# AppleHolic/pytorch_sound

Hardware: AMD Instinct MI355X
Metric: audio-sec/s STFT+mel+fwd/bwd (higher is better)
Workload: dtype bf16; 1 GPU; configs[1]: Conv1d separator (4 x ResBlock1, C=256, on 513-bin magnitude), 22.05 kHz, STFT 1024/256, 80 mel, batch 32 x 2 s per GPU, Adam, bf16 autocast; global_batch=32, parallelism=dp1, model_params=5520386

## Files before the change

include/psnd.h:

```cpp
#ifndef PSND_H
#define PSND_H

#include <stdint.h>
#include <stddef.h>

#ifdef __cplusplus
extern "C" {
#endif

#define PSND_OK 0
#define PSND_E_ARG (-1)
#define PSND_E_SHAPE (-2)
#define PSND_E_HIP (-3)
#define PSND_E_UNSUPPORTED (-4)

#define PSND_FRAMING_CENTER 0
#define PSND_FRAMING_HIFIGAN 1
#define PSND_FRAMING_NONE 2

int psnd_version(void);
const char *psnd_last_error(void);
#ifdef PSND_LAB
void psnd_env_refresh(void);
#endif
// ... 121 lines not shown
int psnd_convtr1d_cl_fwd(const void *xa, const void *wf, const float *bias_rep, int64_t N, int Lp, int L, int HP, int Cip, int Cr,
                         int stride, int padding, int LpO, int HPO, float act_slope, void *out_raw, void *out_act, void *stream);
int psnd_convtr1d_cl_wgrad_splits(int64_t N, int Lp, int Cip, int Cr, int stride);
int psnd_convtr1d_cl_bwd(const void *g_raw, const void *g_act, const void *act, float act_slope, const void *wb, const void *xa,
                         int64_t N, int Lp, int L, int HP, int Cip, int Cr, int stride, int padding, int LpO, int HPO, void *gx,
                         void *g_eff, float *gw_part, void *stream);
int psnd_convtr1d_wnorm_bwd(const float *gw_part, int splits, const float *v, const float *g, int Cin, int Cout, int K, int stride,
                            int Cr, int Cip, float *gv, float *gg, void *stream);
int psnd_cl_mean_act_fwd(const void *a, const void *b, const void *c, const void *d, int count, float slope, void *out, int64_t n,
                         void *stream);
int psnd_cl_mean_act_bwd(const void *g, const void *y, int count, float slope, void *gin, int64_t n, void *stream);
int psnd_cl_sum2(const void *const *a, int na, void *out_a, const void *const *b, int nb, void *out_b, int64_t n, void *stream);
int psnd_cl_colsum_splits(int64_t rows, int C);
int psnd_cl_colsum(const void *g, int64_t rows, int C, int Lp, int lo, int hi, float *part, float *out, void *stream);
int psnd_conv1d_prep_multi(const void *descs_dev, int n, int total_blocks, int max_row, int which, void *stream);
#define PSND_WNORM_MAX 32
typedef struct psnd_wnorm_desc {
    const float *gw_part, *gbias_part;
    const float *v, *g;
    float *gv, *gg, *gbias;
    int splits, Cout, Cin, k, Cb, Ca;
} psnd_wnorm_desc;
int psnd_conv1d_wnorm_bwd_multi(const psnd_wnorm_desc *descs, int n, void *stream);
int psnd_conv1d_cl_bwd(const void *G1, const void *G2, const void *GM, float g2_slope, const void *wb, const void *xa,
                       int64_t N, int Lp, int L, int HP, int Ca, int Cb, int k, int pad, int dil, void *gx, void *g_out,
                       const void *gx_mask, float gx_mask_slope, const void *gx_res, float *gw_part, float *gbias_part,
                       void *stream);
int psnd_conv1d_cl_pair_bwd_supported(int C, int k, int pad2, int dil2, int pad1, int dil1);
int psnd_conv1d_cl_pair_bwd_splits(int64_t N, int Lp, int C, int k);
int psnd_conv1d_cl_pair_bwd(const void *G, const void *wb2, const void *M1, float m1_slope, void *g_mid, const void *wb1, const void *M2,
                            float m2_slope, const void *res, int64_t N, int Lp, int L, int HP, int C, int k, int pad2, int dil2,
                            int pad1, int dil1, void *gx, const void *xa_a, float *gw_a, float *gb_a, const void *G_b,
                            const void *xa_b, int off_b, int dstep_b, float *gw_b, float *gb_b, void *stream);
int psnd_conv1d_wnorm_bwd(const float *gw_part, const float *gbias_part, int splits, const float *v, const float *g,
                          int Cout, int Cin, int k, int Cb, int Ca, float *gv, float *gg, float *gbias, void *stream);
int psnd_to_cl(const float *x, int64_t N, int C, int64_t T, int Lp, int HP, int Cp, int preop, void *out, void *stream);
int psnd_from_cl_tanh(const void *x, int64_t N, int C, int64_t T, int Lp, int HP, int Cp, float *out, void *stream);
int psnd_to_cl_tanh_bwd(const float *g, const float *out_fwd, int64_t N, int C, int64_t T, int Lp, int HP, int Cp, void *gx, void *stream);
int psnd_from_cl(const void *x, int64_t N, int C, int64_t T, int Lp, int HP, int Cp, float *out, void *stream);
int psnd_mask_head_fwd(const void *y, const float *mag, int64_t N, int C, int64_t T, int Lp, int HP, int Cp, float *est,
                       void *stream);
int psnd_mask_head_bwd(const float *gest, const float *mag, const void *y, int64_t N, int C, int64_t T, int Lp, int HP, int Cp,
                       void *gy, void *stream);

int psnd_linear1x1_fwd(const float *x, const float *w, const float *bias, int64_t N, int Cin, int Cout, int64_t T, int relu, int bf16,
                       float *y, void *stream);
// ... 96 lines not shown
```

pytorch_sound_amd/_lib.py:

```python
import ctypes
import os
import numpy as np

_HERE = os.path.dirname(os.path.abspath(__file__))
LIB_PATH = os.environ.get('PSND_LIB', os.path.join(_HERE, 'libpsnd_hip.so'))

PSND_OK = 0
FRAMING_CENTER = 0
FRAMING_HIFIGAN = 1
FRAMING_NONE = 2
LOG_NONE, LOG_E, LOG_10 = 0, 1, 2

_c = ctypes
_P = _c.c_void_p
_I64 = _c.c_int64
_INT = _c.c_int
_F = _c.c_float
_D = _c.c_double

SIGNATURES = {
    'psnd_version': (_INT, []),
    'psnd_last_error': (_c.c_char_p, []),
    'psnd_event_create': (_P, []),
    'psnd_event_destroy': (_INT, [_P]),
# ... 12 lines not shown
    'psnd_mel_plan_build': (_INT, [_INT, _INT, _P, _P]),
    'psnd_mel_fwd': (_INT, [_P, _I64, _I64, _INT, _INT, _P, _INT, _F, _F, _F, _F, _P, _P, _P]),
    'psnd_mel_bwd': (_INT, [_P, _P, _I64, _I64, _INT, _INT, _P, _INT, _F, _F, _F, _F, _P, _P]),
    'psnd_logmel_fwd': (_INT, [_P, _I64, _I64, _INT, _INT, _INT, _P, _F, _INT, _P, _INT, _F, _F, _F, _F, _P, _P]),
    'psnd_conv1d_cl': (_INT, [_P, _P, _P, _F, _P, _P, _P, _P, _I64, _INT, _INT, _INT, _INT, _INT, _INT, _INT, _INT, _F, _F, _P, _P, _P, _P]),
    'psnd_conv1d_cl_pair_supported': (_INT, [_INT, _INT, _INT, _INT, _INT, _INT]),
    'psnd_conv1d_cl_pair': (_INT, [_P, _P, _P, _P, _F, _F, _P, _P, _P, _P, _F, _P, _I64, _INT, _INT, _INT, _INT, _INT, _INT, _INT, _INT, _INT, _F, _P, _P, _P]),
    'psnd_conv1d_cl_wgrad': (_INT, [_P, _P, _P, _F, _P, _I64, _INT, _INT, _INT, _INT, _INT, _INT, _P, _P, _P, _P]),
    'psnd_conv1d_prep': (_INT, [_P, _P, _P, _INT, _INT, _INT, _INT, _INT, _P, _P, _P, _P]),
    'psnd_conv1d_wnorm_bwd': (_INT, [_P, _P, _INT, _P, _P, _INT, _INT, _INT, _INT, _INT, _P, _P, _P, _P]),
    'psnd_conv1d_cl_bwd': (_INT, [_P, _P, _P, _F, _P, _P, _I64, _INT, _INT, _INT, _INT, _INT, _INT, _INT, _INT, _P, _P, _P, _F, _P, _P, _P, _P]),
    'psnd_conv1d_cl_wgrad_multi_splits': (_INT, [_I64, _INT, _INT, _INT, _INT, _INT]),
    'psnd_conv1d_cl_wgrad_multi': (_INT, [_P, _INT, _I64, _INT, _P]),
    'psnd_nan_flag': (_INT, [_P, _I64, _P, _P]),
    'psnd_conv1d_cl_chain_rows': (_INT, [_INT, _INT, _INT, _P]),
    'psnd_conv1d_cl_chain_plan': (_INT, [_INT, _INT, _INT, _P, _I64, _P]),
    'psnd_conv1d_cl_chain': (_INT, [_P, _P, _P, _INT, _I64, _INT, _INT, _INT, _INT, _INT, _P]),
    'psnd_conv_chain_stats': (None, [_P]),
    'psnd_conv1d_cl_pair_bwd_supported': (_INT, [_INT, _INT, _INT, _INT, _INT, _INT]),
    'psnd_conv1d_cl_pair_bwd_splits': (_INT, [_I64, _INT, _INT, _INT]),
    'psnd_conv1d_cl_pair_bwd': (_INT, [_P, _P, _P, _F, _P, _P, _P, _F, _P, _I64, _INT, _INT, _INT, _INT, _INT, _INT, _INT, _INT, _INT, _P, _P, _P, _P,
                                       _P, _P, _INT, _INT, _P, _P, _P]),
    'psnd_conv1d_wnorm_bwd_multi': (_INT, [_P, _INT, _P]),
    'psnd_conv1d_prep_multi': (_INT, [_P, _INT, _INT, _INT, _INT, _P]),
    'psnd_conv1d_cl_wgrad_splits': (_INT, [_I64, _INT, _INT, _INT, _INT]),
    'psnd_mask_head_l1_blocks': (_I64, [_I64, _I64, _INT]),
    'psnd_masked_l1_blocks': (_I64, [_I64]),
    'psnd_masked_l1_fwd': (_INT, [_P, _P, _P, _I64, _INT, _I64, _P, _P, _P, _P]),
    'psnd_masked_l1_bwd': (_INT, [_P, _P, _P, _I64, _INT, _I64, _P, _P, _P, _P, _P]),
    'psnd_to_cl_nfk': (_INT, [_P, _I64, _INT, _I64, _INT, _INT, _INT, _INT, _P, _P]),
    'psnd_mask_head_l1_blocks_nfk': (_I64, [_I64, _I64, _INT]),
    'psnd_mask_head_l1_fwd_nfk': (_INT, [_P, _P, _P, _I64, _INT, _I64, _INT, _INT, _INT, _P, _P, _P]),
    'psnd_mask_head_l1_bwd_nfk': (_INT, [_P, _P, _P, _P, _P, _P, _F, _I64, _INT, _I64, _INT, _INT, _INT, _P, _P]),
    'psnd_mel_fwd_nfk': (_INT, [_P, _I64, _I64, _INT, _INT, _P, _INT, _F, _F, _F, _F, _P, _P, _P]),
    'psnd_mel_bwd_nfk': (_INT, [_P, _P, _I64, _I64, _INT, _INT, _P, _INT, _F, _F, _F, _F, _P, _P]),
    'psnd_mel_l1_fwd_nfk': (_INT, [_P, _I64, _I64, _INT, _INT, _P, _INT, _F, _F, _F, _F, _P, _P, _P, _P]),
    'psnd_mel_l1_bwd_nfk': (_INT, [_P, _P, _P, _F, _I64, _I64, _INT, _INT, _P, _INT, _F, _F, _F, _F, _P, _P]),
    'psnd_mask_head_l1_fwd': (_INT, [_P, _P, _P, _I64, _INT, _I64, _INT, _INT, _INT, _P, _P, _P]),
    'psnd_mask_head_l1_bwd': (_INT, [_P, _P, _P, _P, _P, _P, _F, _I64, _INT, _I64, _INT, _INT, _INT, _P, _P]),
    'psnd_mel_l1_blocks': (_I64, [_I64, _I64, _INT]),
    'psnd_mel_l1_fwd': (_INT, [_P, _I64, _I64, _INT, _INT, _P, _INT, _F, _F, _F, _F, _P, _P, _P, _P]),
    'psnd_mel_l1_bwd': (_INT, [_P, _P, _P, _F, _I64, _I64, _INT, _INT, _P, _INT, _F, _F, _F, _F, _P, _P]),
    'psnd_l1_loss_combine': (_INT, [_P, _P, _P, _INT, _P, _P, _P]),
    'psnd_conv_stats': (_INT, [_P, _INT]),
    'psnd_conv_pair_stats': (_INT, [_P, _INT]),
    'psnd_convtr1d_prep_multi': (_INT, [_P, _INT, _INT, _P]),
# ... 52 lines not shown
    'psnd_l1_loss_blocks': (_I64, [_I64]),
    'psnd_l1_loss_fwd': (_INT, [_P, _P, _I64, _P, _P, _P]),
    'psnd_l1_loss_bwd': (_INT, [_P, _P, _I64, _P, _P, _P, _P]),
    'psnd_l1_loss_sum_fwd': (_INT, [_P, _P, _P, _P, _INT, _P, _P, _P]),
    'psnd_l1_loss_bwd_w': (_INT, [_P, _P, _I64, _P, _D, _P, _P, _P]),
    'psnd_to_cl': (_INT, [_P, _I64, _INT, _I64, _INT, _INT, _INT, _INT, _P, _P]),
    'psnd_from_cl': (_INT, [_P, _I64, _INT, _I64, _INT, _INT, _INT, _P, _P]),
    'psnd_from_cl_tanh': (_INT, [_P, _I64, _INT, _I64, _INT, _INT, _INT, _P, _P]),
    'psnd_to_cl_tanh_bwd': (_INT, [_P, _P, _I64, _INT, _I64, _INT, _INT, _INT, _P, _P]),
}

_lib = None


class PsndError(RuntimeError):
    pass


class WgradDesc(ctypes.Structure):
    _fields_ = [('g', _P), ('xa', _P), ('gw_part', _P), ('gbias_part', _P), ('off0', _INT), ('dstep', _INT),
                ('Ca', _INT), ('Cb', _INT), ('k', _INT), ('splits', _INT)]


class ChainPair(ctypes.Structure):
    _fields_ = [('W1', _P), ('bias1', _P), ('act1_slope', _F), ('mid_out', _P), ('W2', _P), ('bias2', _P),
                ('off1', _INT), ('dstep1', _INT), ('off2', _INT), ('dstep2', _INT), ('act2_slope', _F), ('out_raw', _P), ('out_act', _P),
                ('M1', _P), ('M2', _P), ('m1_slope', _F), ('m2_slope', _F)]


def lib():
    global _lib
    if _lib is None:
        import torch
        if not os.path.exists(LIB_PATH):
            raise PsndError('libpsnd_hip.so not found at %s - run `python -m pytorch_sound_amd._build` '
                            '(there is no CPU / eager fallback)' % LIB_PATH)
        _lib = _load(LIB_PATH)
    return _lib


def _load(path):
    h = ctypes.CDLL(path)
    for name, (res, args) in SIGNATURES.items():
        fn = getattr(h, name)
        fn.restype = res
        fn.argtypes = args
# ... 85 lines not shown
```

pytorch_sound_amd/cl.py:

```python
import ctypes
import os
from pytorch_sound_amd import _switches as _sw
import weakref

import torch

from . import _lib
from ._lib import lib, check, ptr, stream_ptr

ALIGN_C = 32


def round_up(x, m):
    return (x + m - 1) // m * m


class CLShape:

    def __init__(self, N, L, HP):
        self.N, self.L, self.HP = int(N), int(L), int(HP)
        self.Lp = round_up(self.L + 2 * self.HP, 8)

    @property
    def R(self):
# ... 923 lines not shown

        def grad_out(i, v32, g32, Cb):
            gv = gg = gb = None
            if sink is not None and prefs is not None:
                pv, pg, pb = prefs[3 * i:3 * i + 3]
                gv, gg = sink.dest(pv, pv.numel()), sink.dest(pg, pg.numel())
                gb = sink.dest(pb, Cb) if pb is not None else None
                early[i] = [(0, pv) if gv is not None else None, (1, pg) if gg is not None else None,
                            (2, pb) if gb is not None else None]
            gv = torch.empty_like(v32) if gv is None else gv.view_as(v32)
            gg = torch.empty_like(g32) if gg is None else gg.view_as(g32)
            gb = torch.empty(Cb, dtype=torch.float32, device=dev) if gb is None else gb
            return gv, gg, gb

        nsec, sides = _sections(dev, shape.N, shape.N * shape.Lp)
        wstreams = _wgrad_streams(dev) if shape.N * shape.Lp <= 8192 else []
        if wstreams:
            nsec, sides = 1, []
        Nh = shape.N // nsec
        plan = []
        skip = -1
        batch = (nsec == 1 and not wstreams and _pair_enabled() and _sw.lab('PSND_CL_BWD_BATCH', '1') == '1'
                 and shape.N * shape.Lp <= 8192)
        wbatch = []
        own_launch = []
        flush_after = {}
        pair_bwd = (nsec == 1 and not wstreams and not batch and _pair_enabled() and _sw.lab('PSND_CL_PAIR_BWD', '1') != '0'
                    and shape.N * shape.Lp <= 8192)
        lag = None
        with torch.cuda.device(dev):
            g_comb = None
            res_pending = None
            def slabs(i, G1, G2, am, inp, S=None):
                Cout, Cin, k, Ca, Cb, dil, pad, slope = steps[i][:8]
                v32, g32 = saved[5 * i + 3], saved[5 * i + 4]
                if S is None:
                    S = lib().psnd_conv1d_cl_wgrad_splits(Nh, shape.Lp, Ca, Cb, k)
                gw = torch.empty((nsec * S, k, Cb, Ca), dtype=torch.float32, device=dev)
                gbp = torch.empty((nsec * S, Cb), dtype=torch.float32, device=dev)
                gv, gg, gb = grad_out(i, v32, g32, Cb)
                descs[i] = struct.pack('<7Q6i', gw.data_ptr(), gbp.data_ptr(), v32.data_ptr(), g32.data_ptr(), gv.data_ptr(),
                                       gg.data_ptr(), gb.data_ptr(), nsec * S, Cout, Cin, k, Cb, Ca)
                keep.extend([gw, gbp, G1, G2])
                grads[3 * i], grads[3 * i + 1] = gv, gg
                grads[3 * i + 2] = gb[:Cout] if steps[i][9] else None
                return ('w', G1, G2, am, slope, inp, Ca, Cb, k, -pad, dil, gw, gbp, S)
# ... 41 lines not shown
                        wbatch.append((i - 1, g_h, inp1, -pad1, d1))
                        flush_after[id(gx)] = len(wbatch)
                    else:
                        plan.append(('side',) + slabs(i - 1, g_h, None, None, inp1))
                    keep.extend([g_h, gx])
                    res_pending = G
                    g_comb = gx
                    skip = i - 1
                    continue
                if g_comb is None:
                    if g_raw is None and g_act is None:
                        raise _lib.PsndError('CL conv chain backward: no incoming gradient')
                    G1, G2 = g_raw, g_act
                    am = act if g_act is not None else None
                    need_gout = has_res and g_act is not None
                else:
                    G1, G2, am, need_gout = g_comb, None, None, False
                S = lib().psnd_conv1d_cl_wgrad_splits(Nh, shape.Lp, Ca, Cb, k)
                gw = torch.empty((nsec * S, k, Cb, Ca), dtype=torch.float32, device=dev)
                gbp = torch.empty((nsec * S, Cb), dtype=torch.float32, device=dev)
                gv, gg, gb = None, None, None
                g_out = torch.empty((shape.N, shape.Lp, Cb), dtype=torch.bfloat16, device=dev) if need_gout else None
                g_here = g_out if need_gout else G1
                wb_ok = batch and G2 is None and not need_gout and _sw.lab('PSND_CL_BWD_BATCH_ENDS', '0') == '1'
                if i == 0 and not (ctx.needs_input_grad[0] or ctx.needs_input_grad[1]):
                    gx = None
                    if wb_ok:
                        wbatch.append((i, G1, inp, -pad, dil))
                        keep.append(G1)
                        if i > 0:
                            g_comb = gx
                        g_raw = g_act = None
                        continue
                    plan.append((('side',) if wstreams else ()) + ('w', G1, G2, am, slope, inp, Ca, Cb, k, -pad, dil, gw, gbp, S))
                    g_raw = g_act = None
                else:
                    gx = torch.empty((shape.N, shape.Lp, Ca), dtype=torch.bfloat16, device=dev)
                    if i == 0:
                        ep_mask, ep_res = None, None
                    elif role == 'c1':
                        ep_mask, ep_res = inp, res_pending
                    elif role == 'r2':
                        ep_mask, ep_res = inp, g_here
                    else:
                        ep_mask, ep_res = inp, None
                    if wb_ok:
                        plan.append(('b', G1, G2, am, slope, wb, inp, Ca, Cb, k, pad, dil, gx, g_out, ep_mask,
# ... 93 lines not shown
                        check(lib().psnd_conv1d_cl_bwd(q(G1), q(G2), q(am), float(slope), ptr(wb), q(inp), Nh, shape.Lp, shape.L,
                                                       shape.HP, Ca, Cb, k, pad, dil, q(gx), q(g_out), q(ep_mask), ep_slope, q(ep_res),
                                                       None if gw is None else ptr(gw[h * S:(h + 1) * S]),
                                                       None if gbp is None else ptr(gbp[h * S:(h + 1) * S]), st),
                              'psnd_conv1d_cl_bwd')

            st = stream_ptr(dev)
            handed = set()

            def wgrad_batch(part):
                for j0 in range(0, len(part), 32):
                    sub = part[j0:j0 + 32]
                    shp = [(steps[ci][3], steps[ci][4], steps[ci][2]) for ci, _, _, _, _ in sub]
                    main_shape = max(set(shp), key=shp.count)
                    cnt = max(shp.count(main_shape), len(wbatch) // 2) if len(part) < len(wbatch) else shp.count(main_shape)
                    Sb = lib().psnd_conv1d_cl_wgrad_multi_splits(shape.N, shape.Lp, main_shape[0], main_shape[1], main_shape[2], cnt)
                    arr = (_lib.WgradDesc * len(sub))()
                    for d, (ci, G, inp, off0, dstep) in zip(arr, sub):
                        w = slabs(ci, G, None, None, inp, Sb)
                        d.g, d.xa, d.gw_part, d.gbias_part, d.off0, d.dstep = G.data_ptr(), inp.data_ptr(), w[11].data_ptr(), w[12].data_ptr(), off0, dstep
                        d.Ca, d.Cb, d.k, d.splits = steps[ci][3], steps[ci][4], steps[ci][2], Sb
                    check(lib().psnd_conv1d_cl_wgrad_multi(ctypes.addressof(arr), len(sub), shape.N, shape.Lp, st), 'psnd_conv1d_cl_wgrad_multi')

            def finish(convs):
                ds = [descs[ci] for ci in convs]
                for j0 in range(0, len(ds), 32):
                    chunk = ds[j0:j0 + 32]
                    buf = ctypes.create_string_buffer(b''.join(chunk))
                    check(lib().psnd_conv1d_wnorm_bwd_multi(buf, len(chunk), st), 'psnd_conv1d_wnorm_bwd_multi')
                out = []
                for ci in convs:
                    for ent in early.get(ci, ()):
                        if ent is not None:
                            grads[3 * ci + ent[0]] = None
                            out.append(ent[1])
                    handed.add(ci)
                if out:
                    sink.deliver(out)

            if sink is not None and batch and nsec == 1 and not wstreams:
                done_w = 0

                def chunk(part, ready):
                    if part:
                        wgrad_batch(part)
                    finish(ready)

                launches = [e for e in plan if (e[1][-1] if e[0] == 'chainb' else e)[0] == 'pairb']
                L, C = len(launches), max(1, int(HANDOVER_CHUNKS))
                cut = {id(launches[min(L - 1, max(0, round((j + 1) * L / C) - 1))]) for j in range(C - 1)} if L else set()
                ready = []
                for e in plan:
                    run(0, [e])
                    ready += [ci for pe, ci in own_launch if pe is e]
                    last = e[1][-1] if e[0] == 'chainb' else e
                    upto = flush_after.get(id(last[16])) if (last[0] == 'pairb' and id(e) in cut) else None
                    if upto is None:
                        continue
                    part = []
                    if upto is not None and upto > done_w:
                        part = wbatch[done_w:upto]
                        ready += [ci for ci, _, _, _, _ in part]
                        done_w = upto
                    if ready:
                        chunk(part, ready)
                        ready = []
                part = wbatch[done_w:]
                rest = [ci for ci in range(n) if ci not in handed and descs[ci] is not None and ci not in [c for c, _, _, _, _ in part]]
                rest = [ci for ci in rest if ci not in ready]
                if part or rest or ready:
                    chunk(part, ready + rest + [ci for ci, _, _, _, _ in part])
            else:
                _run_sections(dev, nsec, sides, run)
                for sd in set(used):
                    torch.cuda.current_stream(dev).wait_stream(sd)
                wgrad_batch(wbatch)
                finish([ci for ci in range(n) if descs[ci] is not None])
        consume_param_use(ctx)
        return (g_raw, g_act, None, None, None, None, None, None) + tuple(grads)


def _block_node(convs, x, xa, shape, pairs, last_act_slope, want_raw, prep):
    params = []
    for c in convs:
        params += [c.weight_v, c.weight_g, c.bias]
    packs = None if prep is None else _PackList(prep[id(c)] for c in convs)
    if packs is not None:
        packs.owner = prep if isinstance(prep, PrepPacks) else None
    roles = pairs if isinstance(pairs, tuple) else (('c1', 'c2') * (len(convs) // 2) if pairs else ('r2',) * len(convs))
    return ResBlockCL.apply(x, xa, shape, roles, tuple(c.dilation for c in convs), last_act_slope, want_raw, packs, *params)


class _PackList(list):
    owner = None


def _use_block_node(convs, x):
    import os
    return (_sw.lab('PSND_NO_BLOCK_NODE') != '1' and x is not None and len(convs) <= 64
            and all(c.weight_v.shape[0] == c.weight_v.shape[1] for c in convs))


# ... 51 lines not shown
```

pytorch_sound_amd/csrc/psnd_conv.hip:

```cpp
#include "psnd_common.h"
#include "psnd_conv_pair.h"
#include <stdlib.h>
#include <string.h>
#include <atomic>

namespace {

typedef __attribute__((ext_vector_type(8))) short bf16x8;
typedef __attribute__((ext_vector_type(16))) float f32x16;
typedef unsigned short bf16_t;

__device__ __forceinline__ float bf2f(bf16_t v) { return __builtin_bit_cast(float, (unsigned)v << 16); }
__device__ __forceinline__ bf16_t f2bf(float f) {
    unsigned u = __builtin_bit_cast(unsigned, f);
    if ((u & 0x7fffffffu) > 0x7f800000u) return (bf16_t)((u >> 16) | 0x40);
    u += 0x7fffu + ((u >> 16) & 1u);
    return (bf16_t)(u >> 16);
}

typedef __bf16 hwbf16x2 __attribute__((ext_vector_type(2)));
typedef float f32x2_t __attribute__((ext_vector_type(2)));
__device__ __forceinline__ unsigned pack_bf16(float lo, float hi) {
    const f32x2_t v = {lo, hi};
    return __builtin_bit_cast(unsigned, __builtin_convertvector(v, hwbf16x2));
// ... 1235 lines not shown
__global__ __launch_bounds__(1024) void conv_finish_kernel(const float *gw_part, const float *gb_part, int splits, const float *v,
                                                           const float *g, int Cout, int Cin, int k, int Cb, int Ca, float *gv,
                                                           float *gg, float *gbias, unsigned kmagic, unsigned cmagic) {
    extern __shared__ float s_gw[];
    __shared__ float red[32];
    conv_finish_body<MANY>(gw_part, gb_part, splits, v, g, Cin, k, Cb, Ca, gv, gg, gbias, kmagic, cmagic, blockIdx.x, s_gw, red);
}

struct FinishArgs {
    psnd_wnorm_desc d[PSND_WNORM_MAX];
    unsigned kmagic[PSND_WNORM_MAX], cmagic[PSND_WNORM_MAX];
    int blk0[PSND_WNORM_MAX + 1];
    int n;
};
template <bool MANY>
__global__ __launch_bounds__(1024) void conv_finish_multi_kernel(FinishArgs a) {
    extern __shared__ float s_gw[];
    __shared__ float red[32];
    int i = 0;
    while (i + 1 < a.n && (int)blockIdx.x >= a.blk0[i + 1]) ++i;
    const psnd_wnorm_desc &d = a.d[i];
    conv_finish_body<MANY>(d.gw_part, d.gbias_part, d.splits, d.v, d.g, d.Cin, d.k, d.Cb, d.Ca, d.gv, d.gg, d.gbias, a.kmagic[i],
                           a.cmagic[i], (int)blockIdx.x - a.blk0[i], s_gw, red);
}

}

static std::atomic<long long> g_conv_stats[4];
std::atomic<long long> g_conv_pair_stats[4];
extern "C" int psnd_conv_pair_stats(int64_t *out4, int reset) {
    if (out4)
        for (int i = 0; i < 4; ++i) out4[i] = g_conv_pair_stats[i].load();
    if (reset)
        for (int i = 0; i < 4; ++i) g_conv_pair_stats[i].store(0);
    return PSND_OK;
}
extern "C" int psnd_conv_stats(int64_t *out4, int reset) {
    if (out4)
        for (int i = 0; i < 4; ++i) out4[i] = g_conv_stats[i].load();
    if (reset)
        for (int i = 0; i < 4; ++i) g_conv_stats[i].store(0);
    return PSND_OK;
}

static int conv_row_tiles(int64_t R, int Cb, bool with3 = false) {
    const char *fe = PSND_ENV("PSND_CONV_MT");
// ... 567 lines not shown
        if (!d.gw_part || !d.v || !d.g || !d.gv || !d.gg || d.splits < 1 || d.Cout < 1 || d.Cin < 1 || d.k < 1)
            PSND_FAIL(PSND_E_ARG, "conv1d_wnorm_bwd_multi: descriptor %d: null pointer / bad sizes", i);
        const size_t l = sizeof(float) * (size_t)(d.Cin + 1) * d.k;
        if (l > 60 * 1024) PSND_FAIL(PSND_E_SHAPE, "conv1d_wnorm_bwd_multi: Cin*k=%d too large", d.Cin * d.k);
        lds = l > lds ? l : lds;
        a.d[i] = d;
        a.kmagic[i] = (unsigned)((0x100000000ull + (unsigned)d.k - 1) / (unsigned)d.k);
        a.cmagic[i] = (unsigned)((0x100000000ull + (unsigned)d.Cin - 1) / (unsigned)d.Cin);
        a.blk0[i] = total;
        total += d.Cout;
        maxn = d.Cin * d.k > maxn ? d.Cin * d.k : maxn;
        maxsplits = d.splits > maxsplits ? d.splits : maxsplits;
    }
    a.blk0[n] = total;
    const int threads = maxn >= 2048 ? 1024 : 256;
    if (maxsplits > 16)
        hipLaunchKernelGGL(conv_finish_multi_kernel<true>, dim3(total), dim3(1024), lds + 4096, static_cast<hipStream_t>(stream), a);
    else
        hipLaunchKernelGGL(conv_finish_multi_kernel<false>, dim3(total), dim3(threads), lds, static_cast<hipStream_t>(stream), a);
    PSND_CHECK_LAUNCH("conv1d_wnorm_bwd_multi");
    return PSND_OK;
}

namespace {

__global__ __launch_bounds__(256) void convtr_prep_kernel(const float *v, const float *g, const float *bias, int Cin, int Cout, int K, int u,
                                                          int Cr, int Cip, bf16_t *wf, bf16_t *wb, float *bp) {
    __shared__ float red[4];
    const int ci = blockIdx.x, n = Cout * K;
    const float *vr = v + (size_t)ci * n;
    float ss = 0.f;
    for (int i = threadIdx.x; i < n; i += 256) ss += vr[i] * vr[i];
    for (int m = 32; m >= 1; m >>= 1) ss += __shfl_xor(ss, m, 64);
    if ((threadIdx.x & 63) == 0) red[threadIdx.x >> 6] = ss;
    __syncthreads();
    const float scale = g[ci] / __builtin_sqrtf(red[0] + red[1] + red[2] + red[3]);
    const int Nn = u * Cr;
    for (int i = threadIdx.x; i < n; i += 256) {
        const int co = i / K, jk = i - co * K;
        const int tap = jk / u, phi = jk - tap * u;
        const bf16_t w = f2bf(vr[i] * scale);
        wf[pack_index(2, tap, phi * Cr + co, ci, Nn, Cip)] = w;
        wb[pack_index(2, tap, ci, phi * Cr + co, Cip, Nn)] = w;
    }
    if (ci == 0)
        for (int i = threadIdx.x; i < Nn; i += 256) {
// ... 401 lines not shown
```

pytorch_sound_amd/csrc/psnd_core.hip:

```cpp
#include "psnd_common.h"

static thread_local char g_err[512] = "";

void psnd_set_error(const char *fmt, ...) {
    va_list ap;
    va_start(ap, fmt);
    vsnprintf(g_err, sizeof(g_err), fmt, ap);
    va_end(ap);
}

extern "C" int psnd_version(void) { return 137; }

extern "C" const char *psnd_last_error(void) { return g_err; }

#ifdef PSND_LAB
std::atomic<int> g_psnd_env_gen{0};
extern "C" void psnd_env_refresh(void) { g_psnd_env_gen.fetch_add(1, std::memory_order_acq_rel); }
#endif

static inline int64_t pad_of(int n_fft, int hop, int framing) {
    if (framing == PSND_FRAMING_NONE) return 0;
    return framing == PSND_FRAMING_CENTER ? n_fft / 2 : (n_fft - hop) / 2;
}

extern "C" int64_t psnd_frame_count(int64_t T, int n_fft, int hop, int framing) {
    if (T <= 0 || n_fft <= 0 || hop <= 0) return 0;
    const int64_t L = T + 2 * pad_of(n_fft, hop, framing);
    if (L < n_fft) return 0;
    return (L - n_fft) / hop + 1;
}

extern "C" int64_t psnd_frame_sample_index(int64_t f, int m, int64_t T, int n_fft, int hop, int framing) {
    int64_t i = f * hop - pad_of(n_fft, hop, framing) + m;
    if (i < 0) i = -i;
// ... 106 lines not shown
```

Baseline: 97270 audio-s/s.

## Fuse batched conv1d weight-gradient with weight-norm backward in one kernel

Adds a new HIP kernel that computes the split-K weight-gradient slabs for a batch of k=3 channels-last convs with MFMA, then lets the last-arriving block per output tile (found through an atomic counter) run the weight-norm backward reduction in the same launch. Standalone finish blocks handle convs without a wgrad part. The Python backward routes the batched wgrad plus finish work through this path by default when shapes qualify, and also enables batching of end convs under those limits. This removes separate wgrad and wnorm-finish launches and their serialization, at the cost of a persistent counter buffer and shape restrictions.

Result: slower. 93790 audio-s/s, median of 2 (-3.6%).

```diff
diff --git a/include/psnd.h b/include/psnd.h
--- a/include/psnd.h
+++ b/include/psnd.h
@@ -167,6 +167,16 @@
     int splits, Cout, Cin, k, Cb, Ca;
 } psnd_wnorm_desc;
 int psnd_conv1d_wnorm_bwd_multi(const psnd_wnorm_desc *descs, int n, void *stream);
+#define PSND_WGRAD_WN_MAX 28
+typedef struct psnd_wgrad_wn_desc {
+    const void *g, *xa;
+    float *gw_part, *gbias_part;
+    const float *v, *g_w;
+    float *gv, *gg, *gbias;
+    int off0, dstep, Cout, Cin, k, Cb, Ca, splits;
+} psnd_wgrad_wn_desc;
+int psnd_conv1d_cl_wgrad_wn_splits(int64_t N, int Lp, int ci_tiles);
+int psnd_conv1d_cl_wgrad_wn(const psnd_wgrad_wn_desc *d, int n, int64_t N, int Lp, unsigned *counters, void *stream);
 int psnd_conv1d_cl_bwd(const void *G1, const void *G2, const void *GM, float g2_slope, const void *wb, const void *xa,
                        int64_t N, int Lp, int L, int HP, int Ca, int Cb, int k, int pad, int dil, void *gx, void *g_out,
                        const void *gx_mask, float gx_mask_slope, const void *gx_res, float *gw_part, float *gbias_part,
diff --git a/pytorch_sound_amd/_lib.py b/pytorch_sound_amd/_lib.py
--- a/pytorch_sound_amd/_lib.py
+++ b/pytorch_sound_amd/_lib.py
@@ -58,6 +58,8 @@
     'psnd_conv1d_cl_pair_bwd': (_INT, [_P, _P, _P, _F, _P, _P, _P, _F, _P, _I64, _INT, _INT, _INT, _INT, _INT, _INT, _INT, _INT, _INT, _P, _P, _P, _P,
                                        _P, _P, _INT, _INT, _P, _P, _P]),
     'psnd_conv1d_wnorm_bwd_multi': (_INT, [_P, _INT, _P]),
+    'psnd_conv1d_cl_wgrad_wn_splits': (_INT, [_I64, _INT, _INT]),
+    'psnd_conv1d_cl_wgrad_wn': (_INT, [_P, _INT, _I64, _INT, _P, _P]),
     'psnd_conv1d_prep_multi': (_INT, [_P, _INT, _INT, _INT, _INT, _P]),
     'psnd_conv1d_cl_wgrad_splits': (_INT, [_I64, _INT, _INT, _INT, _INT]),
     'psnd_mask_head_l1_blocks': (_I64, [_I64, _I64, _INT]),
@@ -156,6 +158,11 @@
                 ('Ca', _INT), ('Cb', _INT), ('k', _INT), ('splits', _INT)]
 
 
+class WgradWnDesc(ctypes.Structure):
+    _fields_ = [('g', _P), ('xa', _P), ('gw_part', _P), ('gbias_part', _P), ('v', _P), ('g_w', _P), ('gv', _P), ('gg', _P), ('gbias', _P),
+                ('off0', _INT), ('dstep', _INT), ('Cout', _INT), ('Cin', _INT), ('k', _INT), ('Cb', _INT), ('Ca', _INT), ('splits', _INT)]
+
+
 class ChainPair(ctypes.Structure):
     _fields_ = [('W1', _P), ('bias1', _P), ('act1_slope', _F), ('mid_out', _P), ('W2', _P), ('bias2', _P),
                 ('off1', _INT), ('dstep1', _INT), ('off2', _INT), ('dstep2', _INT), ('act2_slope', _F), ('out_raw', _P), ('out_act', _P),
diff --git a/pytorch_sound_amd/cl.py b/pytorch_sound_amd/cl.py
--- a/pytorch_sound_amd/cl.py
+++ b/pytorch_sound_amd/cl.py
@@ -969,6 +969,8 @@
         skip = -1
         batch = (nsec == 1 and not wstreams and _pair_enabled() and _sw.lab('PSND_CL_BWD_BATCH', '1') == '1'
                  and shape.N * shape.Lp <= 8192)
+        wn = (batch and _sw.lab('PSND_CL_WGRAD_WN', '1') == '1'
+              and all(s_[2] == 3 and s_[1] <= 1024 and (s_[10] == 'tail' or (s_[4] <= 256 and 2 * abs(s_[5]) <= 16)) for s_ in steps))
         wbatch = []
         own_launch = []
         flush_after = {}
@@ -1056,7 +1058,8 @@
                 gv, gg, gb = None, None, None
                 g_out = torch.empty((shape.N, shape.Lp, Cb), dtype=torch.bfloat16, device=dev) if need_gout else None
                 g_here = g_out if need_gout else G1
-                wb_ok = batch and G2 is None and not need_gout and _sw.lab('PSND_CL_BWD_BATCH_ENDS', '0') == '1'
+                wb_ok = batch and G2 is None and not need_gout and ((Cb <= 256 and Ca <= 256 and 2 * abs(dil) <= 16) if wn
+                                                                    else _sw.lab('PSND_CL_BWD_BATCH_ENDS', '0') == '1')
                 if i == 0 and not (ctx.needs_input_grad[0] or ctx.needs_input_grad[1]):
                     gx = None
                     if wb_ok:
@@ -1196,8 +1199,26 @@
                         d.Ca, d.Cb, d.k, d.splits = steps[ci][3], steps[ci][4], steps[ci][2], Sb
                     check(lib().psnd_conv1d_cl_wgrad_multi(ctypes.addressof(arr), len(sub), shape.N, shape.Lp, st), 'psnd_conv1d_cl_wgrad_multi')
 
-            def finish(convs):
-                ds = [descs[ci] for ci in convs]
+            S_wn = lib().psnd_conv1d_cl_wgrad_wn_splits(shape.N, shape.Lp, sum((steps[e[0]][3] + 255) // 256 for e in wbatch)) if wn and wbatch else 0
+
+            def wgrad_wn(part, fin):
+                items = [(e[0], e) for e in part] + [(ci, None) for ci in fin]
+                ctr = _wn_counters(dev)
+                for j0 in range(0, len(items), _WN_MAX):
+                    sub = items[j0:j0 + _WN_MAX]
+                    arr = (_lib.WgradWnDesc * len(sub))()
+                    for d, (ci, e) in zip(arr, sub):
+                        if e is not None:
+                            slabs(ci, e[1], None, None, e[2], S_wn)
+                            d.g, d.xa, d.off0, d.dstep = e[1].data_ptr(), e[2].data_ptr(), e[3], e[4]
+                        gw, gbp, v32, g32, gv, gg, gb, S, Cout, Cin, k, Cb, Ca = struct.unpack('<7Q6i', descs[ci])
+                        d.gw_part, d.gbias_part, d.v, d.g_w, d.gv, d.gg, d.gbias = gw, gbp, v32, g32, gv, gg, gb
+                        d.Cout, d.Cin, d.k, d.Cb, d.Ca, d.splits = Cout, Cin, k, Cb, Ca, S
+                    check(lib().psnd_conv1d_cl_wgrad_wn(ctypes.addressof(arr), len(sub), shape.N, shape.Lp, ctr.data_ptr(), st),
+                          'psnd_conv1d_cl_wgrad_wn')
+
+            def finish(convs, launch=True):
+                ds = [descs[ci] for ci in convs] if launch else []
                 for j0 in range(0, len(ds), 32):
                     chunk = ds[j0:j0 + 32]
                     buf = ctypes.create_string_buffer(b''.join(chunk))
@@ -1216,6 +1237,10 @@
                 done_w = 0
 
                 def chunk(part, ready):
+                    if wn:
+                        wgrad_wn(part, [ci for ci in ready if ci not in {e[0] for e in part}])
+                        finish(ready, launch=False)
+                        return
                     if part:
                         wgrad_batch(part)
                     finish(ready)
@@ -1248,10 +1273,29 @@
                 _run_sections(dev, nsec, sides, run)
                 for sd in set(used):
                     torch.cuda.current_stream(dev).wait_stream(sd)
-                wgrad_batch(wbatch)
-                finish([ci for ci in range(n) if descs[ci] is not None])
+                if wn:
+                    wgrad_wn(wbatch, [ci for ci in range(n) if descs[ci] is not None])
+                    finish([ci for ci in range(n) if descs[ci] is not None], launch=False)
+                else:
+                    wgrad_batch(wbatch)
+                    finish([ci for ci in range(n) if descs[ci] is not None])
         consume_param_use(ctx)
         return (g_raw, g_act, None, None, None, None, None, None) + tuple(grads)
+
+
+_WN_MAX = 28
+_WN_COUNTERS = {}
+
+
+def _wn_counters(dev):
+    key = (dev.index, torch.cuda.current_stream(dev).cuda_stream)
+    t = _WN_COUNTERS.get(key)
+    if t is None and torch.cuda.is_current_stream_capturing():
+        t = _WN_COUNTERS.get(dev.index)
+    if t is None:
+        t = _WN_COUNTERS[key] = torch.zeros(4 * _WN_MAX, dtype=torch.int32, device=dev)
+        _WN_COUNTERS.setdefault(dev.index, t)
+    return t
 
 
 def _block_node(convs, x, xa, shape, pairs, last_act_slope, want_raw, prep):
diff --git a/pytorch_sound_amd/csrc/psnd_conv.hip b/pytorch_sound_amd/csrc/psnd_conv.hip
--- a/pytorch_sound_amd/csrc/psnd_conv.hip
+++ b/pytorch_sound_amd/csrc/psnd_conv.hip
@@ -1281,6 +1281,318 @@
     const psnd_wnorm_desc &d = a.d[i];
     conv_finish_body<MANY>(d.gw_part, d.gbias_part, d.splits, d.v, d.g, d.Cin, d.k, d.Cb, d.Ca, d.gv, d.gg, d.gbias, a.kmagic[i],
                            a.cmagic[i], (int)blockIdx.x - a.blk0[i], s_gw, red);
+}
+
+constexpr int WN_MAX = PSND_WGRAD_WN_MAX;
+constexpr int WN_XR = 48;
+constexpr int WN_GP = 96, WN_XP = 288;
+constexpr int WN_STAGE = 32 * WN_GP + WN_XR * WN_XP;
+constexpr int WN_EP = 256 + 4;
+constexpr int kWgradWnLdsBytes = 2 * WN_STAGE * (int)sizeof(bf16_t);
+static_assert(64 * WN_EP * 4 <= kWgradWnLdsBytes, "one tap's 64 x 256 slab tile fits the chunk buffers");
+constexpr int WN_QMAX = 4;
+constexpr int WN_RPP = 2;
+constexpr int WN_WD = 4;
+constexpr int WN_AUX_SC1 = 16;
+struct WgradWnArgs {
+    long long R;
+    int n, nunits, ncompute;
+    int ub0[WN_MAX + 1];
+    int fb0[WN_MAX + 1];
+    int rps[WN_MAX];
+    unsigned *counters;
+    psnd_wgrad_wn_desc d[WN_MAX];
+};
+template <int P>
+__device__ __forceinline__ bf16x8 tr_frag_p(const bf16_t *p0) {
+    const v4s_t a = __builtin_amdgcn_ds_read_tr16_b64_v4i16((v4s_t __attribute__((address_space(3))) *)(p0));
+    const v4s_t b = __builtin_amdgcn_ds_read_tr16_b64_v4i16((v4s_t __attribute__((address_space(3))) *)(p0 + 4 * P));
+    return __builtin_shufflevector(a, b, 0, 1, 2, 3, 4, 5, 6, 7);
+}
+__device__ __forceinline__ void wn_tile(const psnd_wgrad_wn_desc &d, const long long R, const int rps, const int cot, const int cit,
+                                        const int split, bf16_t *sT) {
+    const int tid = threadIdx.x, wave = tid >> 6, lane = tid & 63, li = lane & 31, kg = lane >> 5;
+    const int co0 = cot * 64, ci0 = cit * 256, Ca = d.Ca, Cb = d.Cb;
+    const long long rs = (long long)split * rps, re = min(rs + rps, R);
+    const bool gthr = tid < 256;
+    const int grr = (tid >> 3) & 31, gcg = tid & 7;
+    const int xrr = tid >> 5, xcg = tid & 31;
+    const bool gok = gthr && co0 + 8 * gcg < Cb, xok = ci0 + 8 * xcg < Ca;
+    const bool do_bias = cit == 0 && d.gbias_part != nullptr;
+    const int lo = min(d.off0, d.off0 + 2 * d.dstep), hi = max(d.off0, d.off0 + 2 * d.dstep);
+    const int xrows = 32 + hi - lo;
+    int toff[3];
+#pragma unroll
+    for (int j = 0; j < 3; ++j) toff[j] = d.off0 + j * d.dstep - lo;
+    constexpr unsigned OOB = 0xffffffffu;
+    const __amdgpu_buffer_rsrc_t rG = make_uniform_rsrc(d.g, (int)((size_t)R * Cb * sizeof(bf16_t)));
+    const __amdgpu_buffer_rsrc_t rX = make_uniform_rsrc(d.xa, (int)((size_t)R * Ca * sizeof(bf16_t)));
+    auto ld16 = [&](__amdgpu_buffer_rsrc_t r, unsigned off) __attribute__((always_inline)) {
+        return __builtin_bit_cast(uint4, __builtin_amdgcn_raw_buffer_load_b128(r, (int)off, 0, 0));
+    };
+    f32x16 acc[2][3];
+#pragma unroll
+    for (int m = 0; m < 2; ++m)
+#pragma unroll
+        for (int j = 0; j < 3; ++j)
+#pragma unroll
+            for (int i = 0; i < 16; ++i) acc[m][j][i] = 0.f;
+    float bsum[8] = {0.f, 0.f, 0.f, 0.f, 0.f, 0.f, 0.f, 0.f};
+    uint4 vg[WN_WD], vx[WN_WD][3];
+    auto fetch = [&](auto sc, long long r0) __attribute__((always_inline)) {
+        constexpr int s = decltype(sc)::value;
+        const long long r = r0 + grr;
+        vg[s] = ld16(rG, (r < re && gok) ? (unsigned)(((size_t)r * Cb + co0 + 8 * gcg) * sizeof(bf16_t)) : OOB);
+#pragma unroll
+        for (int u = 0; u < 3; ++u) {
+            const int xi = xrr + 16 * u;
+            const long long rx = r0 + lo + xi;
+            const bool ok = xi < xrows && rx >= 0 && rx < R && xok;
+            vx[s][u] = ld16(rX, ok ? (unsigned)(((size_t)rx * Ca + ci0 + 8 * xcg) * sizeof(bf16_t)) : OOB);
+        }
+    };
+    auto stage = [&](auto sc, bf16_t *sG, bf16_t *sX) __attribute__((always_inline)) {
+        constexpr int s = decltype(sc)::value;
+        if (gthr) {
+            if (do_bias) {
+                const unsigned *pg4 = reinterpret_cast<const unsigned *>(&vg[s]);
+#pragma unroll
+                for (int e = 0; e < 8; ++e) bsum[e] += bf2f((bf16_t)((pg4[e >> 1] >> (16 * (e & 1))) & 0xffff));
+            }
+            *reinterpret_cast<uint4 *>(sG + grr * WN_GP + 8 * gcg) = vg[s];
+        }
+#pragma unroll
+        for (int u = 0; u < 3; ++u) *reinterpret_cast<uint4 *>(sX + (xrr + 16 * u) * WN_XP + 8 * xcg) = vx[s][u];
+    };
+    const int trow = 8 * kg + ((lane & 15) >> 2), tcol = 16 * ((lane >> 4) & 1) + 4 * (lane & 3);
+    const int nchunk = ((int)((re - rs + 31) / 32) + WN_WD - 1) / WN_WD * WN_WD;
+    static_for<0, WN_WD>([&](auto sc) __attribute__((always_inline)) { fetch(sc, rs + 32ll * decltype(sc)::value); });
+    for (int c = 0; c < nchunk; c += WN_WD) {
+        static_for<0, WN_WD>([&](auto sc) __attribute__((always_inline)) {
+            constexpr int s = decltype(sc)::value;
+            const int ch = c + s;
+            bf16_t *sG = sT + (ch & 1) * WN_STAGE, *sX = sG + 32 * WN_GP;
+            stage(sc, sG, sX);
+            __syncthreads();
+            fetch(sc, rs + 32ll * (ch + WN_WD));
+            bf16x8 fa[2][2], fb[2][3];
+#pragma unroll
+            for (int kk = 0; kk < 2; ++kk) {
+#pragma unroll
+                for (int m = 0; m < 2; ++m) fa[kk][m] = tr_frag_p<WN_GP>(sG + (16 * kk + trow) * WN_GP + 32 * m + tcol);
+#pragma unroll
+                for (int j = 0; j < 3; ++j) fb[kk][j] = tr_frag_p<WN_XP>(sX + (16 * kk + trow + toff[j]) * WN_XP + 32 * wave + tcol);
+            }
+#pragma unroll
+            for (int kk = 0; kk < 2; ++kk)
+#pragma unroll
+                for (int m = 0; m < 2; ++m)
+#pragma unroll
+                    for (int j = 0; j < 3; ++j) acc[m][j] = __builtin_amdgcn_mfma_f32_32x32x16_bf16(fa[kk][m], fb[kk][j], acc[m][j], 0, 0, 0);
+        });
+    }
+    __syncthreads();
+    float *sE = reinterpret_cast<float *>(sT);
+    const __amdgpu_buffer_rsrc_t rW = make_uniform_rsrc(d.gw_part, (int)((size_t)d.splits * 3 * Cb * Ca * sizeof(float)));
+#pragma unroll
+    for (int j = 0; j < 3; ++j) {
+        if (j > 0) __syncthreads();
+#pragma unroll
+        for (int m = 0; m < 2; ++m)
+#pragma unroll
+            for (int rg = 0; rg < 16; ++rg) sE[(32 * m + (rg & 3) + 8 * (rg >> 2) + 4 * kg) * WN_EP + 32 * wave + li] = acc[m][j][rg];
+        __syncthreads();
+#pragma unroll
+        for (int u = 0; u < 8; ++u) {
+            const int idx = tid + 512 * u, row = idx >> 6, c4 = 4 * (idx & 63);
+            const int co = co0 + row, ci = ci0 + c4;
+            const bool ok = co < Cb && ci < Ca;
+            const f32x4 v = *reinterpret_cast<const f32x4 *>(sE + row * WN_EP + c4);
+            __builtin_amdgcn_raw_buffer_store_b128(__builtin_bit_cast(u32x4, v), rW,
+                                                   ok ? (int)((((size_t)split * 3 + j) * Cb + co) * Ca + ci) * (int)sizeof(float) : (int)OOB, 0,
+                                                   WN_AUX_SC1);
+        }
+    }
+    __syncthreads();
+    if (do_bias) {
+        float *sb = reinterpret_cast<float *>(sT);
+        if (gthr) {
+#pragma unroll
+            for (int e = 0; e < 8; ++e) {
+                float v = bsum[e];
+#pragma unroll
+                for (int m = 32; m >= 8; m >>= 1) v += __shfl_xor(v, m, 64);
+                if ((lane >> 3) == 0) sb[wave * 64 + 8 * gcg + e] = v;
+            }
+        }
+        __syncthreads();
+        if (tid < 64) {
+            const float v = (sb[tid] + sb[64 + tid]) + (sb[128 + tid] + sb[192 + tid]);
+            const __amdgpu_buffer_rsrc_t rB = make_uniform_rsrc(d.gbias_part, (int)((size_t)d.splits * Cb * sizeof(float)));
+            __builtin_amdgcn_raw_buffer_store_b32(__builtin_bit_cast(unsigned, v), rB,
+                                                  co0 + tid < Cb ? (int)(((size_t)split * Cb + co0 + tid) * sizeof(float)) : (int)OOB, 0, WN_AUX_SC1);
+        }
+    }
+}
+__device__ __forceinline__ void wn_finish(const psnd_wgrad_wn_desc &d, const int cot) {
+    const int tid = threadIdx.x, wave = tid >> 6, lane = tid & 63;
+    const int co0 = cot * 64, S = d.splits, Cin = d.Cin, Ca = d.Ca, Cb = d.Cb;
+    const int nq = (Cin + 255) / 256;
+    const bool v4 = (Cin & 3) == 0;
+    constexpr unsigned OOB = 0xffffffffu;
+    const __amdgpu_buffer_rsrc_t rW = make_uniform_rsrc(d.gw_part, (int)((size_t)S * 3 * Cb * Ca * sizeof(float)));
+    __builtin_amdgcn_fence(__ATOMIC_ACQUIRE, "wavefront");
+    if (tid < 64 && d.gbias && d.gbias_part) {
+        const int co = co0 + tid;
+        const __amdgpu_buffer_rsrc_t rB = make_uniform_rsrc(d.gbias_part, (int)((size_t)S * Cb * sizeof(float)));
+        float b = 0.f;
+        for (int s = 0; s < S; ++s)
+            b += __builtin_bit_cast(float, __builtin_amdgcn_raw_buffer_load_b32(rB, co < d.Cout ? (int)(((size_t)s * Cb + co) * sizeof(float)) : (int)OOB, 0,
+                                                                                 WN_AUX_SC1));
+        if (co < d.Cout) d.gbias[co] = b;
+    }
+    auto load = [&](const int r0, const int q, f32x4 (&G)[WN_RPP][3], float (&V)[WN_RPP][12]) __attribute__((always_inline)) {
+        const int ci = 4 * (lane + 64 * q);
+#pragma unroll
+        for (int r = 0; r < WN_RPP; ++r)
+#pragma unroll
+            for (int j = 0; j < 3; ++j) G[r][j] = f32x4{0.f, 0.f, 0.f, 0.f};
+        for (int s = 0; s < S; s += 2) {
+            f32x4 t[2][WN_RPP][3];
+#pragma unroll
+            for (int h = 0; h < 2; ++h)
+#pragma unroll
+                for (int r = 0; r < WN_RPP; ++r)
+#pragma unroll
+                    for (int j = 0; j < 3; ++j) {
+                        const int co = co0 + r0 + r, sp = s + h < S ? s + h : s;
+                        const bool ok = co < d.Cout && ci < Cin;
+                        t[h][r][j] = __builtin_bit_cast(f32x4, __builtin_amdgcn_raw_buffer_load_b128(
+                                                                   rW, ok ? (int)((((size_t)sp * 3 + j) * Cb + co) * Ca + ci) * (int)sizeof(float) : (int)OOB, 0,
+                                                                   WN_AUX_SC1));
+                    }
+#pragma unroll
+            for (int r = 0; r < WN_RPP; ++r)
+#pragma unroll
+                for (int j = 0; j < 3; ++j) {
+                    G[r][j] += t[0][r][j];
+                    if (s + 1 < S) G[r][j] += t[1][r][j];
+                }
+        }
+#pragma unroll
+        for (int r = 0; r < WN_RPP; ++r) {
+            const int co = co0 + r0 + r;
+            const float *vr = d.v + (size_t)co * Cin * 3 + 3 * ci;
+            if (v4) {
+                const bool ok = co < d.Cout && ci < Cin;
+#pragma unroll
+                for (int u = 0; u < 3; ++u) {
+                    const f32x4 x = ok ? *reinterpret_cast<const f32x4 *>(vr + 4 * u) : f32x4{0.f, 0.f, 0.f, 0.f};
+#pragma unroll
+                    for (int e = 0; e < 4; ++e) V[r][4 * u + e] = x[e];
+                }
+            } else {
+#pragma unroll
+                for (int e = 0; e < 12; ++e) V[r][e] = (co < d.Cout && ci + e / 3 < Cin) ? vr[e] : 0.f;
+            }
+        }
+    };
+    auto store = [&](const int r0, const int q, const f32x4 (&G)[WN_RPP][3], const float (&V)[WN_RPP][12], const float (&gs)[WN_RPP],
+                     const float (&sv)[WN_RPP]) __attribute__((always_inline)) {
+        const int ci = 4 * (lane + 64 * q);
+#pragma unroll
+        for (int r = 0; r < WN_RPP; ++r) {
+            const int co = co0 + r0 + r;
+            if (co >= d.Cout || ci >= Cin) continue;
+            float o[12];
+#pragma unroll
+            for (int e = 0; e < 12; ++e) o[e] = gs[r] * (G[r][e % 3][e / 3] - V[r][e] * sv[r]);
+            float *dst = d.gv + (size_t)co * Cin * 3 + 3 * ci;
+            if (v4) {
+#pragma unroll
+                for (int u = 0; u < 3; ++u) *reinterpret_cast<f32x4 *>(dst + 4 * u) = f32x4{o[4 * u], o[4 * u + 1], o[4 * u + 2], o[4 * u + 3]};
+            } else {
+#pragma unroll
+                for (int e = 0; e < 12; ++e)
+                    if (ci + e / 3 < Cin) dst[e] = o[e];
+            }
+        }
+    };
+    for (int r0 = WN_RPP * wave; r0 < 64; r0 += 8 * WN_RPP) {
+        if (co0 + r0 >= d.Cout) break;
+        f32x4 G[WN_RPP][3];
+        float V[WN_RPP][12], ss[WN_RPP], dot[WN_RPP];
+#pragma unroll
+        for (int r = 0; r < WN_RPP; ++r) ss[r] = 0.f, dot[r] = 0.f;
+        for (int q = 0; q < nq; ++q) {
+            load(r0, q, G, V);
+#pragma unroll
+            for (int r = 0; r < WN_RPP; ++r)
+#pragma unroll
+                for (int e = 0; e < 12; ++e) {
+                    ss[r] = __builtin_fmaf(V[r][e], V[r][e], ss[r]);
+                    dot[r] = __builtin_fmaf(V[r][e], G[r][e % 3][e / 3], dot[r]);
+                }
+        }
+        float gs[WN_RPP], sv[WN_RPP];
+#pragma unroll
+        for (int r = 0; r < WN_RPP; ++r) {
+#pragma unroll
+            for (int m = 32; m >= 1; m >>= 1) {
+                ss[r] += __shfl_xor(ss[r], m, 64);
+                dot[r] += __shfl_xor(dot[r], m, 64);
+            }
+            const int co = co0 + r0 + r;
+            const float inv = 1.f / __builtin_sqrtf(ss[r]);
+            const float dd = dot[r] * inv;
+            gs[r] = co < d.Cout ? d.g_w[co] * inv : 0.f;
+            sv[r] = inv * dd;
+            if (lane == 0 && co < d.Cout) d.gg[co] = dd;
+        }
+        if (nq == 1) {
+            store(r0, 0, G, V, gs, sv);
+        } else {
+            for (int q = 0; q < nq; ++q) {
+                load(r0, q, G, V);
+                store(r0, q, G, V, gs, sv);
+            }
+        }
+    }
+}
+__global__ __launch_bounds__(512, 1) void conv_wgrad_wn_kernel(WgradWnArgs a) {
+    extern __shared__ __attribute__((aligned(16))) bf16_t smem_dyn[];
+    __shared__ int s_last;
+    const int b = (int)blockIdx.x;
+    int i = 0, cot;
+    if (b < a.ncompute) {
+        const int xcd = b & 7, slot = b >> 3;
+        cot = slot & 3;
+        const int u = (slot >> 2) * 8 + xcd;
+        if (u >= a.nunits) return;
+        while (i + 1 < a.n && u >= a.ub0[i + 1]) ++i;
+        const psnd_wgrad_wn_desc &d = a.d[i];
+        if (cot * 64 >= d.Cb) return;
+        const int nct = (d.Ca + 255) / 256, local = u - a.ub0[i];
+        const int split = local / nct, cit = local - split * nct;
+        wn_tile(d, a.R, a.rps[i], cot, cit, split, smem_dyn);
+        asm volatile("s_waitcnt vmcnt(0)" ::: "memory");
+        __syncthreads();
+        if (threadIdx.x == 0) {
+            __attribute__((address_space(1))) unsigned *ctr = (__attribute__((address_space(1))) unsigned *)(a.counters + 4 * i + cot);
+            const unsigned last = (unsigned)(d.splits * nct - 1);
+            const unsigned old = __hip_atomic_fetch_add(ctr, 1u, __ATOMIC_RELAXED, __HIP_MEMORY_SCOPE_AGENT);
+            s_last = old == last;
+            if (old == last) __hip_atomic_store(ctr, 0u, __ATOMIC_RELAXED, __HIP_MEMORY_SCOPE_AGENT);
+        }
+        __syncthreads();
+        if (!s_last) return;
+        wn_finish(d, cot);
+    } else {
+        const int f = b - a.ncompute;
+        if (f >= a.fb0[a.n]) return;
+        while (i + 1 < a.n && f >= a.fb0[i + 1]) ++i;
+        wn_finish(a.d[i], f - a.fb0[i]);
+    }
 }
 
 }
@@ -1894,6 +2206,73 @@
     return PSND_OK;
 }
 
+static int64_t wgrad_wn_rps(int64_t R, int splits) {
+    int64_t rps = (R + splits - 1) / splits;
+    rps = (rps + 31) / 32 * 32;
+    return rps < 64 ? 64 : rps;
+}
+extern "C" int psnd_conv1d_cl_wgrad_wn_splits(int64_t N, int Lp, int ci_tiles) {
+    if (N <= 0 || Lp <= 0 || ci_tiles <= 0) return 0;
+    const int64_t R = N * (int64_t)Lp;
+    int64_t cus = 256;
+    if (const char *e = PSND_ENV("PSND_WGRAD_WN_CUS")) cus = psnd_env_int(e, cus, 32, 65535);
+    int s = 1;
+    for (int t = 2; t <= 16; ++t)
+        if (32 * (((int64_t)ci_tiles * t + 7) / 8) <= cus) s = t;
+    return (int)((R + wgrad_wn_rps(R, s) - 1) / wgrad_wn_rps(R, s));
+}
+
+extern "C" int psnd_conv1d_cl_wgrad_wn(const psnd_wgrad_wn_desc *d, int n, int64_t N, int Lp, unsigned *counters, void *stream) {
+    if (!d || n < 0 || (n > 0 && !counters)) PSND_FAIL(PSND_E_ARG, "conv1d_cl_wgrad_wn: null pointer");
+    if (n == 0) return PSND_OK;
+    if (n > WN_MAX) PSND_FAIL(PSND_E_UNSUPPORTED, "conv1d_cl_wgrad_wn: %d convs (at most %d per launch)", n, WN_MAX);
+    if (N <= 0 || Lp <= 0) PSND_FAIL(PSND_E_SHAPE, "conv1d_cl_wgrad_wn: N=%lld Lp=%d", (long long)N, Lp);
+    const int64_t R = N * (int64_t)Lp;
+    WgradWnArgs a;
+    memset(&a, 0, sizeof(a));
+    a.R = R, a.n = n, a.counters = counters;
+    int units = 0, fin = 0;
+    for (int i = 0; i < n; ++i) {
+        const psnd_wgrad_wn_desc &c = d[i];
+        if (!c.gw_part || !c.v || !c.g_w || !c.gv || !c.gg || c.splits < 1 || c.Cout < 1 || c.Cin < 1 || c.k != 3 || c.Cout > c.Cb ||
+            c.Cin > c.Ca || c.Cin > 256 * WN_QMAX || (c.gbias && !c.gbias_part))
+            PSND_FAIL(PSND_E_ARG, "conv1d_cl_wgrad_wn: conv %d: null pointer / bad sizes (Cout=%d Cin=%d k=%d Cb=%d Ca=%d splits=%d)", i, c.Cout,
+                      c.Cin, c.k, c.Cb, c.Ca, c.splits);
+        if ((size_t)c.splits * 3 * c.Cb * c.Ca * sizeof(float) >= ((size_t)1 << 31))
+            PSND_FAIL(PSND_E_SHAPE, "conv1d_cl_wgrad_wn: conv %d: slabs larger than 2 GB", i);
+        a.d[i] = c;
+        a.ub0[i] = units, a.fb0[i] = fin;
+        if (c.g) {
+            if (!c.xa) PSND_FAIL(PSND_E_ARG, "conv1d_cl_wgrad_wn: conv %d: null input", i);
+            if (c.Cb > 256 || c.Ca % 8 || c.Cb % 8)
+                PSND_FAIL(PSND_E_SHAPE, "conv1d_cl_wgrad_wn: conv %d: Ca=%d Cb=%d (Cb <= 256, multiples of 8)", i, c.Ca, c.Cb);
+            if (2 * (c.dstep < 0 ? -c.dstep : c.dstep) > WN_XR - 32)
+                PSND_FAIL(PSND_E_UNSUPPORTED, "conv1d_cl_wgrad_wn: conv %d: dilation %d: the taps span more than %d rows", i, c.dstep, WN_XR - 32);
+            if ((size_t)R * (size_t)(c.Ca > c.Cb ? c.Ca : c.Cb) * 2 >= ((size_t)1 << 31))
+                PSND_FAIL(PSND_E_SHAPE, "conv1d_cl_wgrad_wn: conv %d: operand larger than 2 GB", i);
+            const int64_t rps = wgrad_wn_rps(R, c.splits);
+            if ((R + rps - 1) / rps != c.splits)
+                PSND_FAIL(PSND_E_SHAPE, "conv1d_cl_wgrad_wn: conv %d: %d row ranges do not cut %lld rows (ask psnd_conv1d_cl_wgrad_wn_splits)", i,
+                          c.splits, (long long)R);
+            a.rps[i] = (int)rps;
+            units += c.splits * ((c.Ca + 255) / 256);
+        } else {
+            fin += (c.Cout + 63) / 64;
+        }
+    }
+    a.ub0[n] = units, a.fb0[n] = fin;
+    a.nunits = units;
+    a.ncompute = 32 * ((units + 7) / 8);
+    {
+        hipError_t e = hipFuncSetAttribute(reinterpret_cast<const void *>(conv_wgrad_wn_kernel), hipFuncAttributeMaxDynamicSharedMemorySize,
+                                           kWgradWnLdsBytes);
+        if (e != hipSuccess) PSND_FAIL(PSND_E_HIP, "conv1d_cl_wgrad_wn: set LDS size: %s", hipGetErrorString(e));
+    }
+    hipLaunchKernelGGL(conv_wgrad_wn_kernel, dim3((unsigned)(a.ncompute + fin)), dim3(512), kWgradWnLdsBytes, static_cast<hipStream_t>(stream), a);
+    PSND_CHECK_LAUNCH("conv1d_cl_wgrad_wn");
+    return PSND_OK;
+}
+
 namespace {
 
 __global__ __launch_bounds__(256) void convtr_prep_kernel(const float *v, const float *g, const float *bias, int Cin, int Cout, int K, int u,
diff --git a/pytorch_sound_amd/csrc/psnd_core.hip b/pytorch_sound_amd/csrc/psnd_core.hip
--- a/pytorch_sound_amd/csrc/psnd_core.hip
+++ b/pytorch_sound_amd/csrc/psnd_core.hip
@@ -9,7 +9,7 @@
     va_end(ap);
 }
 
-extern "C" int psnd_version(void) { return 137; }
+extern "C" int psnd_version(void) { return 138; }
 
 extern "C" const char *psnd_last_error(void) { return g_err; }
 
```
